# thomasneff/AdaNeRF

Hardware: NVIDIA H100
Metric: frames_per_sec_800x800 (higher is better)
Workload: dtype bf16

## Files before the change

adanerf_b200/csrc/mlp.cu:

```cuda
#include <cuda_bf16.h>
#include <cuda_runtime.h>

#include "mlp.cuh"
#include "posenc.cuh"
#include "ptx.cuh"
#include "tiles.cuh"

namespace adn {

template <uint8_t V>
struct ConstFlags {
  __device__ constexpr operator uint8_t() const { return V; }
};

constexpr int kInSlots = 2;

template <int NSPLIT>
struct MlpCfg {
  static constexpr int kNB = (NSPLIT == 2) ? 4 : 2;
  static constexpr int kStageBytes = kBlkBytes;
  __host__ __device__ static constexpr int stages(int n_blk) { return NSPLIT == 2 ? 5 : (n_blk > 2 ? 6 : 8); }
  __host__ __device__ static constexpr size_t in_bytes(int n_blk) {
    return NSPLIT == 2 ? size_t(NSPLIT) * kNB * kBlkBytes : size_t(kInSlots) * n_blk * kBlkBytes;
  }
  __host__ __device__ static constexpr int n_bars(int n_blk) { return 2 * stages(n_blk) + (NSPLIT == 1 ? 2 * kInSlots : 2); }
  __host__ __device__ static constexpr size_t smem_bytes(int n_blk) {
    return in_bytes(n_blk) + size_t(stages(n_blk)) * kStageBytes + size_t(kSideFloats) * 4 + size_t(n_bars(n_blk)) * 8 +
           1024 ;
  }
  static constexpr size_t kMaxSmemBytes = smem_bytes(2) > smem_bytes(3) ? smem_bytes(2) : smem_bytes(3);
};
static_assert(MlpCfg<1>::kMaxSmemBytes <= 232448 && MlpCfg<2>::kMaxSmemBytes <= 232448, "shared memory per block (sm_90)");

__device__ __forceinline__ void encode_row(const EncodeParams& enc, long long i, long long rows, uint8_t* blk, int row,
                                           bool view) {
  const TileFormat act{1, 2, {0, 64, 0}, {64, 64, 0}};
  const int n_p = 3 + 6 * enc.sc.n_freq_pos;
  zero_row(act, blk, uint32_t(row), 0, view ? 1 : shading_p_blocks(n_p));
  if (i < rows) {
    long long ray;
    float zw;
    if (enc.ray_idx) {
      ray = enc.ray_idx[i];
      zw = enc.z[i];
    } else {
      ray = i / enc.K;
      zw = enc.zlut_dense[i - ray * enc.K];
    }
    float pos[3], dir[3];
    sample_inputs(enc.sc, false, enc.ray_o, enc.ray_d, ray, zw, pos, dir);
    auto put = [&](int j, float v) { put_feature(act, blk, j >> 6, uint32_t(row), j & 63, v); };
    if (view) posenc3_rt(dir, enc.sc.n_freq_dir, put);
    else posenc3_rt(pos, enc.sc.n_freq_pos, put);
  }
}

template <int NSPLIT, bool ENC>
__global__ void __launch_bounds__(kMlpThreads, 1)
mlp_kernel(const __grid_constant__ MlpProgram prog, const uint8_t* __restrict__ wblob, const uint8_t* __restrict__ in_tiles,
           float* __restrict__ out, const long long* __restrict__ rows_dev, long long rows_host, int* err_flag,
           const __grid_constant__ EncodeParams enc) {
  static_assert(!ENC || NSPLIT == 1, "fused input encoder: shading net (plain bf16) only");
  using Cfg = MlpCfg<NSPLIT>;
  constexpr int NB = Cfg::kNB;
  const int STAGES = Cfg::stages(prog.in.n_blk);
  constexpr int STAGE_BYTES = Cfg::kStageBytes;
  constexpr int STAGE_K = stage_k_steps(NSPLIT);
  constexpr int kConsumerWarps = 8, kProducerWarp = 8;
  constexpr int kEncThreads = 96;
  constexpr int kConsumerRegs = ENC ? 232 : 240, kProducerRegs = ENC ? 40 : 24;
  static_assert(2 * kConsumerRegs + kProducerRegs <= 3 * 168, "registers the launch allocates");

  extern __shared__ uint8_t smem_raw[];
  uint8_t* smem = smem_raw + ((1024u - (smem_u32(smem_raw) & 1023u)) & 1023u);
  uint8_t* act = smem;
  uint8_t* ring = act + Cfg::in_bytes(prog.in.n_blk);
  float* side = reinterpret_cast<float*>(ring + size_t(STAGES) * STAGE_BYTES);
  uint64_t* w_full = reinterpret_cast<uint64_t*>(side + kSideFloats);
  uint64_t* w_empty = w_full + STAGES;
  uint64_t* in_full = w_empty + STAGES;
  uint64_t* in_empty = in_full + kInSlots;

  const int warp = __shfl_sync(0xffffffffu, int(threadIdx.x >> 5), 0);
  const int lane = threadIdx.x & 31;
  const long long rows = rows_dev ? *rows_dev : rows_host;
  const long long n_tiles = (rows + kTileM - 1) / kTileM;

  for (int i = threadIdx.x; i < kSideFloats; i += blockDim.x) side[i] = prog.side[i];
  if (threadIdx.x == 0) {
    for (int s = 0; s < STAGES; ++s) {
      mbar_init(&w_full[s], 1);
      mbar_init(&w_empty[s], kConsumerWarps);
    }
    if (NSPLIT == 1) {
      for (int s = 0; s < kInSlots; ++s) {
        mbar_init(&in_full[s], ENC ? kEncThreads : 1);
        mbar_init(&in_empty[s], kConsumerWarps);
      }
    } else {
      for (int g = 0; g < 2; ++g) mbar_init(&in_full[g], 1);
    }
    mbar_fence_init();
  }
  __syncthreads();

  if (warp >= kProducerWarp) {
    setmaxnreg_dec<kProducerRegs>();
    if (NSPLIT == 1 && warp > kProducerWarp) {
      if (!ENC && !(warp == kProducerWarp + 1 && lane == 0)) return;
      const uint32_t tile_bytes = prog.in.tile_bytes();
      int slot = 0;
      uint32_t phase = 0;
      for (long long t = blockIdx.x; t < n_tiles; t += gridDim.x) {
        mbar_wait(&in_empty[slot], phase ^ 1, err_flag, 3);
        uint8_t* dst = act + size_t(slot) * tile_bytes;
        if constexpr (ENC) {
          for (int task = int(threadIdx.x) - 32 * (kProducerWarp + 1); task < 2 * kTileM; task += kEncThreads) {
            const int row = task & (kTileM - 1);
            const bool view = task >= kTileM;
            encode_row(enc, t * kTileM + row, rows, dst + (view ? prog.in_nblk0 : 0) * kBlkBytes, row, view);
          }
          fence_proxy_async_smem();
          mbar_arrive(&in_full[slot]);
        } else {
          mbar_arrive_expect_tx(&in_full[slot], tile_bytes);
          bulk_g2s(dst, in_tiles + size_t(t) * tile_bytes, tile_bytes, &in_full[slot]);
        }
        if (++slot == kInSlots) {
          slot = 0;
          phase ^= 1;
        }
      }
      return;
    }
    if (warp == kProducerWarp && lane == 0) {
      int stage = 0;
      uint32_t phase = 0;
      for (long long t = blockIdx.x; t < n_tiles; t += gridDim.x) {
        for (int l = 0; l < prog.n_layers; ++l) {
          const MlpLayer& L = prog.layers[l];
          const int n_st = layer_stages(L, NSPLIT);
          for (int i = 0; i < n_st; ++i) {
            mbar_wait(&w_empty[stage], phase ^ 1, err_flag, 1);
            mbar_arrive_expect_tx(&w_full[stage], STAGE_BYTES);
            bulk_g2s(ring + size_t(stage) * STAGE_BYTES, wblob + L.w_off + size_t(i) * STAGE_BYTES, STAGE_BYTES, &w_full[stage]);
            if (++stage == STAGES) {
              stage = 0;
              phase ^= 1;
            }
          }
        }
      }
    }
    return;
  }

  setmaxnreg_inc<kConsumerRegs>();
  const int wg = warp >> 2;
  const int tw = threadIdx.x & 127;
  const int r0 = 64 * wg + 16 * (warp & 3) + (lane >> 2);
  const int cq = 2 * (lane & 3);
  const int bar_id = 1 + wg;
  const uint32_t act_s = smem_u32(act);
  const uint32_t ring_s = smem_u32(ring);
  const uint32_t wg_off = uint32_t(wg) * (kBlkBytes / 2);
  uint32_t in_s = act_s;
  auto blk_addr = [&](int term, int blk) -> uint32_t { return in_s + uint32_t(term * NB + blk) * kBlkBytes; };
  const uint64_t desc_hi = make_desc_sw128(0) & ~uint64_t(0x3FFF);
  auto desc = [&](uint32_t addr) -> uint64_t { return desc_hi | uint64_t((addr & 0x3FFFF) >> 4); };
  const uint64_t desc64_hi = make_desc_sw64(0) & ~uint64_t(0x3FFF);
  auto desc64 = [&](uint32_t addr) -> uint64_t { return desc64_hi | uint64_t((addr & 0x3FFFF) >> 4); };

  uint32_t afrag[4][4][4];
  auto clear_afrag = [&](int kb0, int kb1) {
#pragma unroll
    for (int kb = 0; kb < 4; ++kb)
#pragma unroll
      for (int k = 0; k < 4; ++k)
#pragma unroll
        for (int j = 0; j < 4; ++j)
          if (kb >= kb0 && kb < kb1) afrag[kb][k][j] = 0u;
  };

  int stage = 0;
  uint32_t phase = 0;
  int prev = -1;
  auto k_block = [&](bool first, int nk, auto mma) {
    mbar_wait(&w_full[stage], phase, err_flag, 2);
    wgmma_fence();
    const uint32_t b = ring_s + uint32_t(stage) * STAGE_BYTES;
#pragma unroll
    for (int k = 0; k < STAGE_K; ++k) {
      if (k < nk) mma(k, b, (first && k == 0) ? 0u : 1u);
    }
    wgmma_commit();
    wgmma_wait<1>();
    if (prev >= 0 && lane == 0) mbar_arrive(&w_empty[prev]);
    prev = stage;
    if (++stage == STAGES) {
      stage = 0;
      phase ^= 1;
    }
  };

  auto fetch_input = [&](long long tt) {
    if (tw != 0) return;
    const uint8_t* src = in_tiles + size_t(tt) * prog.in.tile_bytes() + wg_off;
    mbar_arrive_expect_tx(&in_full[wg], uint32_t(NSPLIT * prog.in_nblk0) * (kBlkBytes / 2));
    for (int term = 0; term < NSPLIT; ++term)
      for (int b = 0; b < prog.in_nblk0; ++b)
        bulk_g2s(act + size_t(term * NB + b) * kBlkBytes + wg_off, src + prog.in.blk_off(term, b), kBlkBytes / 2, &in_full[wg]);
  };
  if (NSPLIT == 2 && blockIdx.x < n_tiles) fetch_input(blockIdx.x);

  int in_slot = 0;
  uint32_t in_phase = 0;
  for (long long t = blockIdx.x; t < n_tiles; t += gridDim.x) {
    if constexpr (NSPLIT == 2) {
      mbar_wait(&in_full[wg], in_phase, err_flag, 4);
      in_phase ^= 1;
    } else {
      mbar_wait(&in_full[in_slot], in_phase, err_flag, 4);
      in_s = act_s + uint32_t(in_slot) * prog.in.tile_bytes();
      clear_afrag(0, 4);
    }
    float alpha[2] = {0.0f, 0.0f};
    for (int l = 0; l < prog.n_layers; ++l) {
      const MlpLayer& L = prog.layers[l];
      float acc[2][64];
#pragma unroll
      for (int nh = 0; nh < 2; ++nh) {
        if (nh >= L.n_half) break;
        if (NSPLIT == 2) {
          for (int kb = 0; kb < L.n_kb; ++kb) {
            for (int k0 = 0; k0 < L.k_cnt[kb]; k0 += STAGE_K) {
              const uint32_t a_hi = blk_addr(0, kb) + wg_off + 32 * k0;
              const uint32_t a_lo = a_hi + uint32_t(NB) * kBlkBytes;
              k_block(kb == 0 && k0 == 0, L.k_cnt[kb] - k0, [&](int k, uint32_t b_hi, uint32_t accumulate) {
                const uint32_t b_lo = b_hi + uint32_t(kBlkBytes / 2);
                wgmma_m64n128_bf16(acc[nh], desc(a_hi + 32 * k), desc64(b_hi + 32 * k), accumulate);
                wgmma_m64n128_bf16(acc[nh], desc(a_lo + 32 * k), desc64(b_hi + 32 * k), 1u);
                wgmma_m64n128_bf16(acc[nh], desc(a_hi + 32 * k), desc64(b_lo + 32 * k), 1u);
              });
            }
          }
        } else {
          auto from_smem = [&](int blk) {
            const uint32_t a = blk_addr(0, blk) + wg_off;
            return [&, a](int k, uint32_t b, uint32_t accumulate) {
              wgmma_m64n128_bf16(acc[nh], desc(a + 32 * k), desc(b + 32 * k), accumulate);
            };
          };
#pragma unroll
          for (int ib = 0; ib < NB; ++ib) {
            if (ib >= L.in_first) break;
            k_block(ib == 0, L.k_cnt[ib], from_smem(ib));
          }
#pragma unroll
          for (int hb = 0; hb < 4; ++hb) {
            if (hb >= L.n_hid) break;
            k_block(hb == 0 && L.in_first == 0, 4, [&](int k, uint32_t b, uint32_t accumulate) {
              wgmma_m64n128_bf16_rs(acc[nh], afrag[hb][k], desc(b + 32 * k), accumulate);
            });
          }
          if (L.in_last) k_block(L.n_kb == 1, L.k_cnt[L.n_kb - 1], from_smem(prog.in_nblk0));
        }
      }
      wgmma_wait<0>();
      if (lane == 0) mbar_arrive(&w_empty[prev]);
      prev = -1;
      const bool fetch_next = l + 1 == prog.n_layers && t + gridDim.x < n_tiles;
      const bool fetch_early = fetch_next && !(L.flags & LF_OUT_ACT);
      if constexpr (NSPLIT == 2) {
        named_bar_sync(bar_id, 128);
        if (fetch_early) fetch_input(t + gridDim.x);
      } else {
        if (l + 1 == prog.n_layers && lane == 0) mbar_arrive(&in_empty[in_slot]);
      }

      auto epilogue = [&](auto flags) {
        float rgb[2][3] = {{0.f, 0.f, 0.f}, {0.f, 0.f, 0.f}};
        if (NSPLIT == 1 && !(flags & LF_OUT_ACT)) clear_afrag(0, 4);
#pragma unroll
        for (int nh = 0; nh < 2; ++nh) {
          if (nh >= L.n_half) {
            if (NSPLIT == 1 && (flags & LF_OUT_ACT)) clear_afrag(2 * nh, 4);
            break;
          }
#pragma unroll
          for (int i = 0; i < 16; ++i) {
            const int col = nh * 128 + 8 * i + cq;
            const float2 b = *reinterpret_cast<const float2*>(side + L.bias_off + col);
#pragma unroll
            for (int rr = 0; rr < 2; ++rr) {
              const int row = r0 + 8 * rr;
              float v0 = acc[nh][4 * i + 2 * rr] + b.x;
              float v1 = acc[nh][4 * i + 2 * rr + 1] + b.y;
              if (flags & LF_FINAL_RAW) {
                const long long grow = t * kTileM + row;
                if (grow < rows) *reinterpret_cast<float2*>(out + grow * prog.out_cols + col) = make_float2(v0, v1);
                continue;
              }
              if (flags & LF_RELU) {
                v0 = fmaxf(v0, 0.0f);
                v1 = fmaxf(v1, 0.0f);
              }
              if (flags & LF_ALPHA_DOT) {
                const float2 w = *reinterpret_cast<const float2*>(side + prog.alpha_w_off + col);
                alpha[rr] = fmaf(v1, w.y, fmaf(v0, w.x, alpha[rr]));
              }
              if (flags & LF_OUT_ACT) {
                const uint32_t hi = bf16x2(v0, v1);
                if (NSPLIT == 1) {
                  afrag[2 * nh + (i >> 3)][(i >> 1) & 3][2 * (i & 1) + rr] = hi;
                } else {
                  const uint32_t off = uint32_t(col >> 6) * kBlkBytes + sw128_offset(uint32_t(row), uint32_t(col & 63));
                  *reinterpret_cast<uint32_t*>(act + off) = hi;
                  *reinterpret_cast<uint32_t*>(act + NB * kBlkBytes + off) = bf16x2_lo(v0, v1, hi);
                }
              }
              if (flags & LF_FINAL_RGB) {
#pragma unroll
                for (int k = 0; k < 3; ++k) {
                  const float2 w = *reinterpret_cast<const float2*>(side + prog.rgb_w_off + k * 128 + col);
                  rgb[rr][k] = fmaf(v1, w.y, fmaf(v0, w.x, rgb[rr][k]));
                }
              }
            }
          }
        }
        if (flags & LF_FINAL_RGB) {
#pragma unroll
          for (int rr = 0; rr < 2; ++rr) {
            float a = alpha[rr], c0 = rgb[rr][0], c1 = rgb[rr][1], c2 = rgb[rr][2];
#pragma unroll
            for (int m = 1; m <= 2; m <<= 1) {
              a += __shfl_xor_sync(0xffffffffu, a, m);
              c0 += __shfl_xor_sync(0xffffffffu, c0, m);
              c1 += __shfl_xor_sync(0xffffffffu, c1, m);
              c2 += __shfl_xor_sync(0xffffffffu, c2, m);
            }
            const long long grow = t * kTileM + r0 + 8 * rr;
            if ((lane & 3) == 0 && grow < rows)
              reinterpret_cast<float4*>(out)[grow] = make_float4(c0 + side[prog.rgb_b_off], c1 + side[prog.rgb_b_off + 1],
                                                                 c2 + side[prog.rgb_b_off + 2], a + side[prog.alpha_b_off]);
          }
        }
      };
      using F = uint8_t;
      constexpr F kEpiFlags = LF_RELU | LF_ALPHA_DOT | LF_OUT_ACT | LF_FINAL_RAW | LF_FINAL_RGB;
      switch (L.flags & kEpiFlags) {
        case LF_RELU | LF_OUT_ACT: epilogue(ConstFlags<LF_RELU | LF_OUT_ACT>{}); break;
        case LF_RELU | LF_OUT_ACT | LF_ALPHA_DOT: epilogue(ConstFlags<LF_RELU | LF_OUT_ACT | LF_ALPHA_DOT>{}); break;
        case LF_OUT_ACT: epilogue(ConstFlags<LF_OUT_ACT>{}); break;
        case LF_RELU | LF_FINAL_RGB: epilogue(ConstFlags<LF_RELU | LF_FINAL_RGB>{}); break;
        case LF_FINAL_RAW: epilogue(ConstFlags<LF_FINAL_RAW>{}); break;
        default: epilogue(F(L.flags)); break;
      }
      if constexpr (NSPLIT == 2) {
        fence_proxy_async_smem();
        named_bar_sync(bar_id, 128);
        if (fetch_next && !fetch_early) fetch_input(t + gridDim.x);
      }
    }
    if (NSPLIT == 1 && ++in_slot == kInSlots) {
      in_slot = 0;
      in_phase ^= 1;
    }
  }
}

__global__ void pack_rows_kernel(const float* __restrict__ x, long long rows_host, const long long* __restrict__ rows_dev,
                                 int n_feat, const __grid_constant__ TileFormat fmt, uint8_t* __restrict__ tiles) {
  const long long rows = rows_dev ? *rows_dev : rows_host;
  const long long n_tiles = (rows + kTileM - 1) / kTileM;
  const long long total = n_tiles * kTileM * fmt.n_blk * 8;
  for (long long i = blockIdx.x * (long long)blockDim.x + threadIdx.x; i < total; i += (long long)gridDim.x * blockDim.x) {
    const int chunk = int(i & 7);
    const long long rb = i >> 3;
    const int blk = int(rb % fmt.n_blk);
    const long long row = rb / fmt.n_blk;
    const long long t = row >> 7;
    pack_tile_chunk(fmt, tiles + size_t(t) * fmt.tile_bytes(), blk, uint32_t(row & (kTileM - 1)), chunk,
                    [&](int c) { return row < rows ? x[row * n_feat + c] : 0.0f; });
  }
}

cudaError_t set_max_dyn_smem_once(const void* func, int bytes, unsigned long long* done) {
  int dev = 0;
  cudaError_t e = cudaGetDevice(&dev);
  if (e != cudaSuccess) return e;
  if (dev < 64 && ((__atomic_load_n(done, __ATOMIC_ACQUIRE) >> dev) & 1ull)) return cudaSuccess;
  e = cudaFuncSetAttribute(func, cudaFuncAttributeMaxDynamicSharedMemorySize, bytes);
  if (e != cudaSuccess) return e;
  if (dev < 64) __atomic_fetch_or(done, 1ull << dev, __ATOMIC_RELEASE);
  return cudaSuccess;
}

template <int NSPLIT, bool ENC>
static cudaError_t launch_mlp_t(const MlpProgram& prog, const uint8_t* wblob, const uint8_t* in_tiles, float* out,
                                const long long* rows_dev, long long rows_host, int* err_flag, int num_sms, cudaStream_t stream,
                                const EncodeParams& enc) {
  static unsigned long long attr_done = 0;
  if (prog.in.n_blk < 1 || prog.in.n_blk > 3) return cudaErrorInvalidValue;
  const size_t smem = MlpCfg<NSPLIT>::smem_bytes(prog.in.n_blk);
  auto kernel = mlp_kernel<NSPLIT, ENC>;
  cudaError_t e = set_max_dyn_smem_once(reinterpret_cast<const void*>(kernel), int(MlpCfg<NSPLIT>::kMaxSmemBytes), &attr_done);
  if (e != cudaSuccess) return e;
  long long grid = num_sms;
  if (!rows_dev) {
    const long long n_tiles = (rows_host + kTileM - 1) / kTileM;
    if (n_tiles < grid) grid = n_tiles < 1 ? 1 : n_tiles;
  }
  kernel<<<unsigned(grid), kMlpThreads, smem, stream>>>(prog, wblob, in_tiles, out, rows_dev, rows_host, err_flag, enc);
  return cudaGetLastError();
}

cudaError_t launch_mlp(const MlpProgram& prog, const uint8_t* wblob, const uint8_t* in_tiles, float* out,
                       const long long* rows_dev, long long rows_host, int* err_flag, int num_sms, cudaStream_t stream,
                       const EncodeParams* enc) {
  if (enc) {
    if (prog.in.n_terms != 1) return cudaErrorInvalidValue;
    return launch_mlp_t<1, true>(prog, wblob, in_tiles, out, rows_dev, rows_host, err_flag, num_sms, stream, *enc);
  }
  if (prog.in.n_terms == 2) return launch_mlp_t<2, false>(prog, wblob, in_tiles, out, rows_dev, rows_host, err_flag, num_sms, stream, EncodeParams{});
  return launch_mlp_t<1, false>(prog, wblob, in_tiles, out, rows_dev, rows_host, err_flag, num_sms, stream, EncodeParams{});
}

cudaError_t launch_pack_rows(const float* x, long long rows, const long long* rows_dev, int n_feat, const TileFormat& fmt,
                             uint8_t* tiles, int num_sms, cudaStream_t stream) {
  long long work = ((rows + kTileM - 1) / kTileM) * kTileM * fmt.n_blk * 8;
  int grid = int((work + 255) / 256);
  if (grid < 1) grid = 1;
  if (grid > 16 * num_sms) grid = 16 * num_sms;
  pack_rows_kernel<<<grid, 256, 0, stream>>>(x, rows, rows_dev, n_feat, fmt, tiles);
  return cudaGetLastError();
}

}
```

Measured before the change: 79.41.

## Stagger warpgroup 1 behind warpgroup 0 on weight ring and specialize k-step counts

Adds a per-stage 'lead' mbarrier that warpgroup 0 arrives on after issuing its wgmmas. Before each long layer, warpgroup 1 waits until warpgroup 0 is a fixed number of stages ahead, so the two consumer warpgroups are offset in time and contend less for tensor cores and shared-memory bandwidth. The k-step loop is also dispatched to a compile-time count instead of using per-iteration predicates, and empty k-blocks skip the MMA issue entirely. The cost is extra barrier traffic and a deliberate stall on warpgroup 1, plus a risk of deadlock if the lag ever reaches the ring depth.

```diff
diff --git a/adanerf_b200/csrc/mlp.cu b/adanerf_b200/csrc/mlp.cu
--- a/adanerf_b200/csrc/mlp.cu
+++ b/adanerf_b200/csrc/mlp.cu
@@ -1,5 +1,7 @@
 #include <cuda_bf16.h>
 #include <cuda_runtime.h>
+
+#include <type_traits>
 
 #include "mlp.cuh"
 #include "posenc.cuh"
@@ -12,6 +14,16 @@
 struct ConstFlags {
   __device__ constexpr operator uint8_t() const { return V; }
 };
+
+template <int N, class F>
+__device__ __forceinline__ void with_k_steps(int nk, F&& f) {
+  if constexpr (N == 1) {
+    f(std::integral_constant<int, 1>{});
+  } else {
+    if (nk >= N) f(std::integral_constant<int, N>{});
+    else with_k_steps<N - 1>(nk, f);
+  }
+}
 
 constexpr int kInSlots = 2;
 
@@ -23,7 +35,8 @@
   __host__ __device__ static constexpr size_t in_bytes(int n_blk) {
     return NSPLIT == 2 ? size_t(NSPLIT) * kNB * kBlkBytes : size_t(kInSlots) * n_blk * kBlkBytes;
   }
-  __host__ __device__ static constexpr int n_bars(int n_blk) { return 2 * stages(n_blk) + (NSPLIT == 1 ? 2 * kInSlots : 2); }
+  __host__ __device__ static constexpr int n_bars(int n_blk) { return 3 * stages(n_blk) + (NSPLIT == 1 ? 2 * kInSlots : 2); }
+  static constexpr int kLag = 2;
   __host__ __device__ static constexpr size_t smem_bytes(int n_blk) {
     return in_bytes(n_blk) + size_t(stages(n_blk)) * kStageBytes + size_t(kSideFloats) * 4 + size_t(n_bars(n_blk)) * 8 +
            1024 ;
@@ -64,6 +77,8 @@
   using Cfg = MlpCfg<NSPLIT>;
   constexpr int NB = Cfg::kNB;
   const int STAGES = Cfg::stages(prog.in.n_blk);
+  constexpr int LAG = Cfg::kLag;
+  static_assert(LAG < Cfg::stages(2) && LAG < Cfg::stages(3), "warpgroup 0 must never need a ring slot warpgroup 1 holds");
   constexpr int STAGE_BYTES = Cfg::kStageBytes;
   constexpr int STAGE_K = stage_k_steps(NSPLIT);
   constexpr int kConsumerWarps = 8, kProducerWarp = 8;
@@ -78,7 +93,8 @@
   float* side = reinterpret_cast<float*>(ring + size_t(STAGES) * STAGE_BYTES);
   uint64_t* w_full = reinterpret_cast<uint64_t*>(side + kSideFloats);
   uint64_t* w_empty = w_full + STAGES;
-  uint64_t* in_full = w_empty + STAGES;
+  uint64_t* w_lead = w_empty + STAGES;
+  uint64_t* in_full = w_lead + STAGES;
   uint64_t* in_empty = in_full + kInSlots;
 
   const int warp = __shfl_sync(0xffffffffu, int(threadIdx.x >> 5), 0);
@@ -91,6 +107,7 @@
     for (int s = 0; s < STAGES; ++s) {
       mbar_init(&w_full[s], 1);
       mbar_init(&w_empty[s], kConsumerWarps);
+      mbar_init(&w_lead[s], kConsumerWarps / 2);
     }
     if (NSPLIT == 1) {
       for (int s = 0; s < kInSlots; ++s) {
@@ -185,22 +202,34 @@
   int stage = 0;
   uint32_t phase = 0;
   int prev = -1;
+  auto next_stage = [&] {
+    if (++stage == STAGES) {
+      stage = 0;
+      phase ^= 1;
+    }
+  };
   auto k_block = [&](bool first, int nk, auto mma) {
     mbar_wait(&w_full[stage], phase, err_flag, 2);
+    if (nk == 0) {
+      if (lane == 0) {
+        mbar_arrive(&w_empty[stage]);
+        if (wg == 0) mbar_arrive(&w_lead[stage]);
+      }
+      next_stage();
+      return;
+    }
     wgmma_fence();
     const uint32_t b = ring_s + uint32_t(stage) * STAGE_BYTES;
-#pragma unroll
-    for (int k = 0; k < STAGE_K; ++k) {
-      if (k < nk) mma(k, b, (first && k == 0) ? 0u : 1u);
-    }
-    wgmma_commit();
+    with_k_steps<STAGE_K>(nk, [&](auto n) {
+#pragma unroll
+      for (int k = 0; k < decltype(n)::value; ++k) mma(k, b, (first && k == 0) ? 0u : 1u);
+      wgmma_commit();
+    });
+    if (wg == 0 && lane == 0) mbar_arrive(&w_lead[stage]);
     wgmma_wait<1>();
     if (prev >= 0 && lane == 0) mbar_arrive(&w_empty[prev]);
     prev = stage;
-    if (++stage == STAGES) {
-      stage = 0;
-      phase ^= 1;
-    }
+    next_stage();
   };
 
   auto fetch_input = [&](long long tt) {
@@ -227,6 +256,15 @@
     float alpha[2] = {0.0f, 0.0f};
     for (int l = 0; l < prog.n_layers; ++l) {
       const MlpLayer& L = prog.layers[l];
+      if (wg == 1 && layer_stages(L, NSPLIT) > 2 * LAG) {
+        int s = stage + LAG;
+        uint32_t par = phase;
+        if (s >= STAGES) {
+          s -= STAGES;
+          par ^= 1;
+        }
+        mbar_wait(&w_lead[s], par, err_flag, 5);
+      }
       float acc[2][64];
 #pragma unroll
       for (int nh = 0; nh < 2; ++nh) {
```

Result: faster. 81.15, median of 6 (+2.2%).
